# adfriend45/HYBRID9

Hardware: AMD Instinct MI355X
Metric: grid-cell-steps/sec at 0.5° global (1/2/4/8 GPUs) + achieved HBM GB/s (higher is better)
Workload: dtype f32

## Files before the change

hybrid9_amd/csrc/h9g.hip:

```cpp
#include <hip/hip_runtime.h>

#include <math.h>
#include <stdio.h>
#include <stdlib.h>
#include <string.h>

#include <algorithm>
#include <atomic>
#include <mutex>
#include <string>
#include <thread>
#include <vector>

#include "h9g_ctx.h"
#include "h9g_io.h"

static_assert(H9G_ERR_NOSNAP_K == H9G_ERR_NOSNAP, "kernel and ABI error codes");
static_assert(H9G_NDAILY == DAILY_ROWS, "the daily line of the ABI and of h9g_rows.h");

#define H9G_PF_ROWS 32
__global__ void __launch_bounds__(256) h9g_perm_forcing_kernel(int c0, int cend, int cpb, int nt, int n, size_t fvar,
                                                               size_t ds, size_t dvar, const int *__restrict__ perm,
                                                               const float *__restrict__ src, float *__restrict__ dst) {
  const unsigned nb = (unsigned)((cend - c0 + cpb - 1) / cpb), x = blockIdx.x % H9G_NXCD, j = blockIdx.x / H9G_NXCD;
// ... 1009 lines not shown
  for (int k = K_PAIR; k <= K_PROBE; k++)
    for (int j = 0; j < 3 && m < n; j++) out[m++] = ctx->kstat[k][j];
  if (reset)
    for (auto &row : ctx->kstat) row[0] = row[1] = row[2] = 0.0;
  return m;
}

#if defined(H9G_STAMPS)
static int stamps_report(h9g_ctx *ctx) {
  if (ctx->d_stamps && (ctx->kind == K_PAIR || ctx->kind == K_PAIR11 || ctx->kind == K_PAIR1)) {
    const size_t cw = (size_t)shape_info(kind_info(ctx->kind).shape).wave_cols, nw = (ctx->n + cw - 1) / cw;
    std::vector<unsigned> st(8 * nw);
    HIPCHK(hipMemcpy(st.data(), ctx->d_stamps, sizeof(unsigned) * 8 * nw, hipMemcpyDeviceToHost));
    double sum[8] = {0}, tot = 0;
    for (size_t w = 0; w < nw; w++)
      for (int k = 0; k < 8; k++) sum[k] += st[8 * w + k];
    const double steps = (double)nw * days_in_year(ctx->last_year) * ctx->cfg.nisurf;
    fprintf(stderr, "h9g stamps (cycles/wave/substep):");
    for (int k = 0; k < 8; k++) { fprintf(stderr, " p%d=%.0f", k, sum[k] / steps); tot += sum[k]; }
    fprintf(stderr, " total=%.0f\n", tot / steps);
    if (shape_info(ctx->stamp_shape).front()) {
      std::vector<unsigned> fs(8 * nw);
      HIPCHK(hipMemcpy(fs.data(), ctx->d_stamps + 8 * ctx->stamp_blocks, sizeof(unsigned) * 8 * nw, hipMemcpyDeviceToHost));
      double w = 0, f = 0;
      for (size_t k = 0; k < nw; k++) { w += fs[8 * k]; f += fs[8 * k + 1]; }
      fprintf(stderr, "h9g stamps, front waves (cycles/wave/substep): wait at barrier 1=%.0f front=%.0f\n", w / steps,
              f / steps);
    }
    std::vector<double> wt(nw, 0.0);
    for (size_t w = 0; w < nw; w++)
      for (int k = 0; k < 8; k++) wt[w] += st[8 * w + k];
    std::vector<double> ws(wt);
    std::sort(ws.begin(), ws.end());
    const double mean = tot / nw;
    fprintf(stderr, "h9g wave totals / mean: min %.3f p50 %.3f p90 %.3f p99 %.3f max %.3f\n", ws[0] / mean,
            ws[nw / 2] / mean, ws[nw * 9 / 10] / mean, ws[nw * 99 / 100] / mean, ws[nw - 1] / mean);
    double bx[8] = {0}, nx[8] = {0}, bs[4] = {0}, ns[4] = {0};
    for (size_t w = 0; w < nw; w++) {
      const size_t b = w / 4;
      bx[b % 8] += wt[w];
      nx[b % 8] += 1;
      bs[w % 4] += wt[w];
      ns[w % 4] += 1;
    }
    {
      const double cut90 = ws[nw * 9 / 10], cut50 = ws[nw / 2];
      double hi[8] = {0}, lo[8] = {0}, nh = 0, nl = 0;
      for (size_t w = 0; w < nw; w++) {
        if (wt[w] >= cut90) { nh++; for (int k = 0; k < 8; k++) hi[k] += st[8 * w + k]; }
        if (wt[w] <= cut50) { nl++; for (int k = 0; k < 8; k++) lo[k] += st[8 * w + k]; }
// ... 216 lines not shown
```

hybrid9_amd/csrc/h9g_pair.h:

```cpp
#pragma once
#include <type_traits>

#include "h9g_step.h"
#include "h9g_expr.h"
#if !defined(__HIPCC__) && !defined(__HIP__)
#define __device__
#define __forceinline__ inline
#endif

#ifndef H9G_EXACT_HOOK
#define H9G_EXACT_HOOK(k0, ns)
#endif
#if defined(H9G_COUNT_EXACT)
__device__ unsigned long long h9g_exact_count;
__device__ unsigned h9g_exact_wave[1 << 16];
#endif
namespace h9k {

enum : int {
  PF_TS = 0, PF_HKS, PF_BSW, PF_PSI,
  PF_NINVB,
  PF_ITS,
  PF_PTE,
  PF_C3,
// ... 8 lines not shown
  PS_LAI = PS_DAY + D_N,
  PS_LAIL, PS_PM, PS_PFM, PS_PLEN, PS_RDEPTH,
  PS_DR0,
  PS_DRS = PS_DR0 + 4 * DRP_N,
  PS_SVZWT = PS_DR0 + 2 * DR_N,
  PS_SVWA, PS_SVRNF, PS_SVERR, PS_SVNS,
  PS_SVEVAP,
  PS_N
};
enum : int { SV_ZWT = 0, SV_WA, SV_RNF, SV_ERR, SV_NS, SV_EVAP };
static_assert((PS_DAY + D_NUMC) % 2 == 0 && (PS_DAY + D_RAARAC) % 2 == 0 && (PS_DAY + D_DGRAC) % 2 == 0 &&
                  (PS_DAY + D_DRR) % 2 == 0 && (PS_DAY + D_RAC) % 2 == 0 && PS_DR0 % 2 == 0,
              "pair fields must start a row");

#ifndef H9G_EB_FAST
#define H9G_EB_FAST 1
#endif
#ifndef H9G_P1_TASKS
#define H9G_P1_TASKS 7
#endif
#ifndef H9G_P1_FRONT
#define H9G_P1_FRONT 1
#endif
enum : int { ROLE_ALL = 0, ROLE_FRONT = 1, ROLE_MAIN = 2 };
struct FrontRes {
  float qflx_surf, tran, evg, qflx_infl;
};

template <int K>
struct FV {
  float v[K];
};

H9K_HD float sel(int h, float a, float b) { return h ? b : a; }
H9K_HD double seld(int h, double a, double b) { return h ? b : a; }

H9K_HD float pair_swap(float v) {
#if defined(__HIP_DEVICE_COMPILE__)
  const int x = __builtin_bit_cast(int, v);
  return __builtin_bit_cast(float, __builtin_amdgcn_update_dpp(x, x, 0xB1, 0xF, 0xF, false));
#else
  return v;
#endif
}

template <int E>
H9K_HD float pair_bcast(float v) {
// ... 126 lines not shown
#endif
  }
};
#define H9G_PACE_ROWS 16384
__device__ __forceinline__ void pace_key(int &row, int &slot) {
#if defined(__HIP_DEVICE_COMPILE__)
  const unsigned hw = __builtin_amdgcn_s_getreg((31 << 11) | 4);
  const unsigned xcc = __builtin_amdgcn_s_getreg((3 << 11) | 20) & 15u;
  slot = (int)(hw & 15u);
  row = (int)(((((xcc * 8u + ((hw >> 13) & 7u)) * 2u + ((hw >> 12) & 1u)) * 16u + ((hw >> 8) & 15u)) * 4u) +
              ((hw >> 4) & 3u));
#else
  row = slot = 0;
#endif
}

template <int L>
constexpr int pair_resident() { return 3; }

template <int L, int S, int R = pair_resident<L>(), int F = 0>
struct PairStore {
  static constexpr int NT = L / 2;
  static constexpr bool kFront = F != 0;
  static_assert(!kFront || S == 2, "the front wave serves a one-column wave");
  static constexpr bool kRecip = true, kRts = L <= 8 || R <= 2 || S <= 22, kDayRecip = L <= 8 || R <= 2 || S <= 22;
  static constexpr bool kRtsHK = kRts;
  static constexpr int NPF = kRecip ? (kRts ? PF_SVH2O : PF_RTS0) : PF_RPSI0;
  static constexpr int NPS = kDayRecip ? PS_SVZWT : PS_DR0;
  static constexpr int TH0 = (NPF * NT + (NPS + 1) / 2) * S;
  enum : int {
    HO_SMP = TH0 + L, HO_H2O1 = HO_SMP + L, HO_ZWT, HO_GO, HO_PAD,
    HO_SURF, HO_TRAN, HO_EVG, HO_INFL, HO_END
  };
  static_assert((HO_END - TH0 - L) % 2 == 0, "whole rows");
  static constexpr int ROWS = NPF * NT + (NPS + 1) / 2 + (S == 2 ? NT : 0) + (kFront ? (HO_END - HO_SMP) / 2 : 0);
  static constexpr int GBLOCK = 65536;
  lds_float *self, *even;
  const lds_float *zt;
  float *svw;
  static constexpr int RESIDENT = R;
  Pacer pace;
  lds_float *wb;
  static constexpr int LANES = S;
  static constexpr bool kSpare = !(L >= 10 && R >= 3 && S >= 44);
  __device__ __forceinline__ void day_start(int day) const { pace.day_start(day, RESIDENT); }
  __device__ __forceinline__ float zi(int i) const { return zt[i]; }
  __device__ __forceinline__ float zim(int i) const { return zt[L + 2 + i]; }
  __device__ __forceinline__ double rdz_t(int i) const {
    return join_d(zt[2 * (L + 2) + 2 * i], zt[2 * (L + 2) + 2 * i + 1]);
  }
  __device__ __forceinline__ float lay(int p, int i) const {
    return even[(p * NT + ((i - 1) >> 1)) * S + ((i - 1) & 1)];
  }
  __device__ __forceinline__ void set_lay(int p, int i, float v) const {
    even[(p * NT + ((i - 1) >> 1)) * S + ((i - 1) & 1)] = v;
  }
  __device__ __forceinline__ float sc(int k) const { return even[(NPF * NT + (k >> 1)) * S + (k & 1)]; }
  __device__ __forceinline__ void set_sc(int k, float v) const {
// ... 328 lines not shown
    cs.set_lay(PF_NINVB, i, -one / bsw);
    cs.set_lay(PF_ITS, i, one / (ts + tsp));
    const float pte = psi * ts / e;
    cs.set_lay(PF_PTE, i, pte);
    cs.set_lay(PF_C3, i, pte / (g.zi(i) - g.zi(i - 1)));
    if constexpr (CS::kRecip) set_lay_d(cs, PF_RPSI0, i, recip64(-psi));
    if constexpr (CS::kRts) set_lay_d(cs, PF_RTS0, i, recip64(ts));
  }
  float mh = cs.lay(PF_HKS, 1);
  if (cs.lay(PF_HKS, 2) < mh) mh = cs.lay(PF_HKS, 2);
  if (cs.lay(PF_HKS, 3) < mh) mh = cs.lay(PF_HKS, 3);
  cs.set_sc(PS_MH3, mh);
  cs.set_sc(PS_TSDZ1, MAXF(zero, (cs.lay(PF_TS, 1) * g.dz(1))));
}

template <class M, class SP, class CS>
constexpr bool pair1_tasks() {
  if constexpr (H9G_P1_TASKS && SP::kSpare && CS::kSpare && !M::kExact)
    return CS::LANES == 2;
  else
    return false;
}

template <int L, class G, class M, class SP, class CS, class PR = NoProf, int ROLE = ROLE_ALL>
H9K_HD int hydrology_pair(const G &g, CS cs, const SP &sp0, St<L> &s, float &rnf_sum, float &errval,
                          M &m, PR &pr, FrontRes *fr = nullptr) {
  constexpr int NT = L / 2;
  const SP sp = L >= 10 ? sp0.fresh() : sp0;
  const float dt = g.dt();
  constexpr double r1000 = 1.0 / 1000.0;
  float zim[L + 1];
#pragma unroll
  for (int i = 1; i <= L; i++) zim[i] = g.zim(i);
  float *h2o = s.h2o, *smp = s.smp;
  float theta[L + 1];
  cs.launder();
#define TS(i) cs.lay(PF_TS, i)
#define HKS(i) cs.lay(PF_HKS, i)
#define BSW(i) cs.lay(PF_BSW, i)
#define PSI(i) cs.lay(PF_PSI, i)
#define LAYF(F, i) cs.lay(F, i)
#define ROOT(i) cs.lay(PF_ROOTR, i)
#define DC(F) cs.sc(PS_DAY + F)
#define OWN(p) sp.own(cs, p, t, h)

  float w0 = zero;
  if constexpr (ROLE == ROLE_FRONT) {
    theta[1] = m.div_d(h2o[1], g.thk(1), g.rthk(1));
    m.div_fix(theta[1], h2o[1], g.thk(1));
  } else {
  w0 = DC(D_FORC) * dt + s.wa;
  bool bad = false;
#pragma unroll
  for (int i = 1; i <= L; i++) {
    w0 = w0 + h2o[i];
    theta[i] = m.div_d(h2o[i], g.thk(i), g.rthk(i));
    bad |= m.div_bad(theta[i]);
  }
  if (__builtin_expect(bad, 0)) {
    H9G_BR(BR_THETA);
#pragma unroll
    for (int i = 1; i <= L; i++) m.div_fix(theta[i], h2o[i], g.thk(i));
  }
  }
  const float hkdepth = one / 2.5f;
  const float fff = 1.0f / hkdepth;
  const float frac_h2osfc = zero;
  float qflx_surf = zero, tran = zero, evg = zero, qflx_infl = zero;
  if constexpr (ROLE != ROLE_MAIN) {
  const float qflx_top_soil = DC(D_FORC);
  const float fsat = cs.sc(PS_FMAX) * m.expf(-0.5f * fff * s.zwt);
  qflx_surf = fsat * qflx_top_soil;
  float beta = zero;
  {
    float rb[L + 1];
    float *const out[1] = {rb};
    auto qb_x = [&](int t, int h) __attribute__((always_inline)) {
      return sel(h, smp[2 * t + 1] - g.zc(2 * t + 1), smp[2 * t + 2] - g.zc(2 * t + 2));
    };
    auto term = [&](int t, int h, float q) __attribute__((always_inline)) {
      float b = one - q;
      b = MINC(one, b);
      b = MAXF(zero, b);
      return FV<1>{{sp.own(cs, PF_ROOTR, t, h) * b}};
    };
    sp.template par_d<NT, 1, NT>(
        [&](int t, int h, bool &bad) __attribute__((always_inline)) -> FV<1> {
          const float q = m.div_d(qb_x(t, h), -150000.0f, 1.0 / -150000.0);
          bad |= m.div_bad(q);
          return term(t, h, q);
        },
        [&](int t, int h) __attribute__((always_inline)) -> FV<1> {
// ... 111 lines not shown
  tran = ftr.v[0];
  evg = fev.v[0];
  }
  float em1 = m.div(g.dz(1) * (theta[1] - watmin), dt, g.rdt()) - tran * ROOT(1);
  em1 = MAXF(zero, em1);
  evg = MINF(em1, evg);
  pr.flux(evg, tran);
  const float qflx_evap = evg;
  float qflx_in_soil = (one - frac_h2osfc) * (qflx_top_soil - qflx_surf);
  qflx_in_soil = qflx_in_soil - (one - frac_h2osfc) * qflx_evap;
  const float qinmax = (one - fsat) * cs.sc(PS_MH3);
  const float qflx_infl_excess = MAXF(zero, qflx_in_soil - (one - frac_h2osfc) * qinmax);
  qflx_infl = qflx_in_soil - qflx_infl_excess;
  qflx_surf = qflx_surf + qflx_infl_excess;
  }
  if constexpr (ROLE == ROLE_FRONT) {
    *fr = FrontRes{qflx_surf, tran, evg, qflx_infl};
    return 0;
  }
  float zwtmm = 1000.0f * s.zwt;
  const int jwt = jwt_of<L>(s.zwt, zim);
  const bool aq = (jwt == L);
  cs.launder();
  if constexpr (ROLE != ROLE_MAIN) pr.mark(1);

  float zq[L + 2];
  float hk[L + 1], dhkdw[L + 1], dsmpdw[L + 1];
  constexpr bool kTask = pair1_tasks<M, SP, CS>();
  FV<1> p0{{zero}}, p1{{zero}};
  FV<2> eA{{zero, zero}}, eS{{zero, zero}};
  bool picks = true, aq_task = false;
  float c_q[L + 1], c_1[L + 1], c_2[L + 1];
  bool flux_done = false;
  float rc_smp = zero, rc_zq = zero;
  {
    float *const outq[1] = {zq};
    float *const outk[4] = {hk, dhkdw, smp, dsmpdw};
    auto eq_exact = [&](int t, int h) __attribute__((always_inline)) -> FV<1> {
          H9G_BR(BR_EQX);
          const int i0 = 2 * t + 1;
          const int il = i0 + h;
          const float zlo = cs.zi(il - 1), zhi = cs.zi(il);
          const float ts = OWN(PF_TS), psi = OWN(PF_PSI);
          float vol_eq;
          if (zwtmm <= zlo) {
            vol_eq = ts;
          } else {
            const float expo = one + OWN(PF_NINVB);
            auto rp = [&]() __attribute__((always_inline)) {
              return join_d(OWN(PF_RPSI0), OWN(PF_RPSI1));
            };
            const bool inl = (zwtmm < zhi) && (zwtmm > zlo);
            const float n0 = ((-psi) + zwtmm - zlo), ni = (-psi + zwtmm - zhi);
            bool bq = false;
            float b0 = divr_d<CS::kRecip>(m, n0, -psi, rp, bq);
            float bi = divr_d<CS::kRecip>(m, ni, -psi, rp, bq);
            if (__builtin_expect(bq, 0)) {
              divr_fix<CS::kRecip>(m, b0, n0, -psi);
// ... 479 lines not shown
          };
          bool sq = false, sw = false;
          float q2 = divr_d<CS::kRts>(m, xn, TS(L), [&]() { return lay_d(cs, PF_RTS0, L); }, sq);
          float x = xof(q2);
          float pw = m.powf_d(x, -BSW(L), sw);
          if (__builtin_expect(sq | sw, 0)) {
            H9G_BR(BR_AQS);
            divr_fix<CS::kRts>(m, q2, xn, TS(L));
            x = xof(q2);
            pw = m.powf(x, -BSW(L));
          }
          const float z = smp_of(PSI(L), pw);
          return FV<2>{{z, dsmpdw_div(BSW(L), z, x, TS(L))}};
        },
        eA, eS);
  }
  }
  }
  const FV<1> pY = p1;
  zq[L + 1] = aq ? eA.v[0] : zero;
  const float smp1 = eS.v[0], dsmpdw1 = eS.v[1];
  cs.launder();
  pr.mark(3);
  if constexpr (ROLE == ROLE_MAIN) {
    cs.wg_sync();
    qflx_surf = cs.ho(CS::HO_SURF);
    tran = cs.ho(CS::HO_TRAN);
    evg = cs.ho(CS::HO_EVG);
    qflx_infl = cs.ho(CS::HO_INFL);
    pr.flux(evg, tran);
    pr.mark(1);
  }
  const float zcA = 0.5f * (zwtmm + g.zc(L));
  const float dzA = (jwt < L) ? g.dz(L) : zwtmm - g.zc(L);
  cs.launder();
  float dwat2[L + 2], GAM[L + 2];
  float BET = zero;
  double rbet = 0.0;
  int zero_pivot = 0;
  auto row = [&](int i, float am, float bm, float cm, float rm) __attribute__((always_inline)) {
    float x;
    if (i == 1) {
      BET = bm;
      x = rm;
    } else {
      BET = row_bet(am, bm, GAM[i]);
      if (BET == 0.0f && !zero_pivot) zero_pivot = i;
      x = row_x(am, rm, dwat2[i - 1]);
    }
    rbet = recip64(BET);
    dwat2[i] = m.div_d(x, BET, rbet);
    bool bad = m.div_bad(dwat2[i]);
    if (i <= L) {
      GAM[i + 1] = m.div_d(cm, BET, rbet);
      bad |= m.div_bad(GAM[i + 1]);
    }
    if (__builtin_expect(bad, 0)) {
      m.div_fix(dwat2[i], x, BET);
      if (i <= L) m.div_fix(GAM[i + 1], cm, BET);
    }
  };
  bool tri_ok = false;
  if constexpr (!M::kExact) {
    bool bad = false, zp = false;
    float qo[L + 1], d1[L + 1], d2[L + 1];
    auto flux3_f = [&](float hki, float num, float dsi, float dsn, float dhk, float den, double rden, int k,
                       bool &b) __attribute__((always_inline)) {
      qo[k] = m.div_d(flux_q(hki, num), den, rden);
      d1[k] = m.div_d(flux_d1(hki, num, dsi, dhk), den, rden);
      d2[k] = m.div_d(flux_d2(hki, num, dsn, dhk), den, rden);
      b |= m.div_bad(qo[k]) | m.div_bad(d1[k]) | m.div_bad(d2[k]);
    };
    if constexpr (kTask && (H9G_P1_TASKS & 2)) {
#pragma unroll
      for (int i = 1; i <= L; i++) {
        qo[i] = c_q[i];
        d1[i] = c_1[i];
        d2[i] = c_2[i];
      }
    }
    if (!kTask || __builtin_expect(!flux_done, 0)) {
#pragma unroll
    for (int i = 1; i <= L - 1; i++)
      flux3_f(hk[i], flux_num(smp[i + 1], smp[i], zq[i + 1], zq[i]), dsmpdw[i], dsmpdw[i + 1], dhkdw[i], g.den(i),
              g.rden(i), i, bad);
    qo[L] = d1[L] = d2[L] = zero;
// ... 42 lines not shown
      }
    };
    auto dzdt = [&](float dz) __attribute__((always_inline)) {
      const float q = m.div_d(dz, dt, g.rdt());
      bad |= m.div_bad(q);
      return q;
    };
    const float bm1 = dzdt(g.dz(1)) + d1[1];
    row_f(1, zero, bm1, d2[1], qflx_infl - qo[1] - tran * ROOT(1));
#pragma unroll
    for (int i = 2; i <= L - 1; i++)
      row_f(i, -d1[i - 1], dzdt(g.dz(i)) - d2[i - 1] + d1[i], d2[i], qo[i - 1] - qo[i] - tran * ROOT(i));
    row_f(L, -d1[L - 1], dzdt(g.dz(L)) - d2[L - 1] + (aq ? d1[L] : zero), aq ? d2[L] : zero,
          qo[L - 1] - (aq ? qo[L] : zero) - tran * ROOT(L));
    const float qA = dzdt(dzA);
    const float bmA = qA - d2[L] + zero;
    const float rmA = qo[L] - zero;
    row_f(L + 1, aq ? -d1[L] : zero, aq ? bmA : qA, zero, aq ? rmA : zero);
    if (__builtin_expect(bad | zp | (bm1 == 0.0f), 0)) {
      H9G_BR(BR_TRISWEEP);
      BET = zero;
      zero_pivot = 0;
      const float bm1x = m.div(g.dz(1), dt, g.rdt()) + d1[1];
      if (bm1x == 0.0f) { errval = bm1x; return 1; }
      row(1, zero, bm1x, d2[1], qflx_infl - qo[1] - tran * ROOT(1));
#pragma unroll
      for (int i = 2; i <= L - 1; i++)
        row(i, -d1[i - 1], m.div(g.dz(i), dt, g.rdt()) - d2[i - 1] + d1[i], d2[i], qo[i - 1] - qo[i] - tran * ROOT(i));
      if (!aq) {
        row(L, -d1[L - 1], m.div(g.dz(L), dt, g.rdt()) - d2[L - 1] + zero, zero, qo[L - 1] - zero - tran * ROOT(L));
        row(L + 1, zero, m.div(dzA, dt, g.rdt()), zero, zero);
      } else {
        row(L, -d1[L - 1], m.div(g.dz(L), dt, g.rdt()) - d2[L - 1] + d1[L], d2[L], qo[L - 1] - qo[L] - tran * ROOT(L));
        row(L + 1, -d1[L], m.div(dzA, dt, g.rdt()) - d2[L] + zero, zero, qo[L] - zero);
      }
      if (zero_pivot) { errval = (float)zero_pivot; return 2; }
    }
    tri_ok = true;
  }
  if (!tri_ok) {
  auto flux3 = [&](float hki, float num, float dsi, float dsn, float dhk, float den, double rden, float &qo,
                   float &d1, float &d2) __attribute__((always_inline)) {
    const float x0 = flux_q(hki, num), x1 = flux_d1(hki, num, dsi, dhk), x2 = flux_d2(hki, num, dsn, dhk);
    qo = m.div_d(x0, den, rden);
    d1 = m.div_d(x1, den, rden);
    d2 = m.div_d(x2, den, rden);
    if (__builtin_expect(m.div_bad(qo) | m.div_bad(d1) | m.div_bad(d2), 0)) {
      m.div_fix(qo, x0, den);
      m.div_fix(d1, x1, den);
      m.div_fix(d2, x2, den);
    }
  };
  float q_prev, dq0_prev, dq1_prev;
  {
    const float den = g.den(1);
    const double rden = g.rden(1);
    const float dzq = (zq[2] - zq[1]);
    const float num = (smp[2] - smp[1]) - dzq;
    float qout, dqodw1, dqodw2;
    flux3(hk[1], num, dsmpdw[1], dsmpdw[2], dhkdw[1], den, rden, qout, dqodw1, dqodw2);
    const float bm1 = m.div(g.dz(1), dt, g.rdt()) + dqodw1;
    if (bm1 == 0.0f) { errval = bm1; return 1; }
    row(1, zero, bm1, dqodw2, qflx_infl - qout - tran * ROOT(1));
    q_prev = qout; dq0_prev = dqodw1; dq1_prev = dqodw2;
  }
#pragma unroll
  for (int i = 2; i <= L - 1; i++) {
    const float den = g.den(i);
    const double rden = g.rden(i);
    const float dzq = zq[i + 1] - zq[i];
    const float num = (smp[i + 1] - smp[i]) - dzq;
    float qout, dqodw1, dqodw2;
    flux3(hk[i], num, dsmpdw[i], dsmpdw[i + 1], dhkdw[i], den, rden, qout, dqodw1, dqodw2);
    row(i, -dq0_prev, m.div(g.dz(i), dt, g.rdt()) - dq1_prev + dqodw1, dqodw2,
        q_prev - qout - tran * ROOT(i));
    q_prev = qout; dq0_prev = dqodw1; dq1_prev = dqodw2;
  }
  {
    constexpr int i = L;
    if (i > jwt) {
      const float qout = zero, dqodw1 = zero;
      row(i, -dq0_prev, m.div(g.dz(i), dt, g.rdt()) - dq1_prev + dqodw1, zero,
          q_prev - qout - tran * ROOT(i));
      row(i + 1, zero, m.div(dzA, dt, g.rdt()), zero, zero);
    } else {
      const float den = zcA - g.zc(i);
      const double rden = recip64(den);
      const float dzq = zq[i + 1] - zq[i];
      const float num = smp1 - smp[i] - dzq;
      float qout, dqodw1, dqodw2;
      flux3(hk[i], num, dsmpdw[i], dsmpdw1, dhkdw[i], den, rden, qout, dqodw1, dqodw2);
      row(i, -dq0_prev, m.div(g.dz(i), dt, g.rdt()) - dq1_prev + dqodw1, dqodw2,
          q_prev - qout - tran * ROOT(i));
      const float qout1 = zero, dqodw1b = zero;
      row(i + 1, -dqodw1, m.div(dzA, dt, g.rdt()) - dqodw2 + dqodw1b, zero, qout - qout1);
    }
  }
  if (zero_pivot) { errval = (float)zero_pivot; return 2; }
  }
#pragma unroll
  for (int i = L; i >= 1; i--) dwat2[i] = dwat2[i] - GAM[i + 1] * dwat2[i + 1];
#pragma unroll
  for (int i = 1; i <= L; i++) h2o[i] = h2o[i] + dwat2[i] * g.dz(i);
  cs.launder();
  pr.mark(4);
  auto s_y_base = [&](int i, float zmm) __attribute__((always_inline)) -> float {
    return one + divr<CS::kRecip>(m, zmm, -cs.lay(PF_PSI, i), [&]() { return lay_d(cs, PF_RPSI0, i); });
  };
  auto s_y_of = [&](int i, float pw) __attribute__((always_inline)) -> float {
    return MAXX(cs.lay(PF_TS, i) * (one - pw), 0.02f);
  };
  auto s_y_at = [&](int i, float zmm) __attribute__((always_inline)) -> float {
    return s_y_of(i, m.powf(s_y_base(i, zmm), cs.lay(PF_NINVB, i)));
  };
  float qcharge, sy_first = zero;
  if (jwt < L) {
    H9G_BR(BR_JWTCOL);
    const int j1 = jwt + 1;
    const float hks_j = cs.lay(PF_HKS, j1);
    float smp_m = zero, zq_m = zero, zc_j = zero;
    if constexpr (kTask && (H9G_P1_TASKS & 2)) {
      smp_m = rc_smp;
      zq_m = rc_zq;
#pragma unroll
      for (int i = 1; i <= L; i++)
        if (i == jwt) zc_j = g.zc(i);
    } else {
#pragma unroll
    for (int i = 1; i <= L; i++) {
      if (i == (jwt > 1 ? jwt : 1)) { smp_m = smp[i]; zq_m = zq[i]; }
      if (i == jwt) zc_j = g.zc(i);
    }
    }
    const float wh_zwt = zero;
    sy_first = s_y_of(jwt + 1, p1.v[0]);
    const float ka = hks_j * p0.v[0];
    const float smp1m = MAXC(smpmin, smp_m);
    const float wh = smp1m - zq_m;
    if (jwt == 0)
      qcharge = -ka * (wh_zwt - wh) / (zwtmm + one);
    else
      qcharge = -ka * (wh_zwt - wh) / ((zwtmm - zc_j) * 2.0f);
    qcharge = MAXC(-10.0f / dt, qcharge);
    qcharge = MINC(10.0f / dt, qcharge);
  } else {
    qcharge = m.div(dwat2[L + 1] * dzA, dt, g.rdt());
  }
  float rous = MAXX(TS(L) * (one - pY.v[0]), 0.02f);
  auto wdiv = [&](float x) __attribute__((always_inline)) {
    if constexpr (!M::kExact) {
      const float q = m.div_d(x, 1000.0f, r1000);
      m.special |= m.div_bad(q);
      return q;
    } else {
      return m.div(x, 1000.0f, r1000);
    }
  };
  int jwt2 = jwt;
  if (jwt == L) {
    s.wa = s.wa + qcharge * dt;
    s.zwt = s.zwt - m.div(qcharge * dt, 1000.0f, r1000) / rous;
  } else {
    float qcharge_tot = qcharge * dt;
    if (qcharge_tot > zero) {
      visit_layers(m, [&](int k) __attribute__((always_inline)) -> bool {
        const int i = jwt + 1 - k;
        const float s_y = k == 0 ? sy_first : s_y_at(i, zwtmm);
        float qcl = MINF(qcharge_tot, s_y * (zwtmm - cs.zi(i - 1)));
        qcl = MAXF(qcl, zero);
        if (s_y > zero) s.zwt = s.zwt - wdiv(qcl / s_y);
        qcharge_tot = qcharge_tot - qcl;
        return !(qcharge_tot <= zero || i == 1);
      });
    } else {
      visit_layers(m, [&](int k) __attribute__((always_inline)) -> bool {
        const int i = jwt + 1 + k;
        const float s_y = k == 0 ? sy_first : s_y_at(i, zwtmm);
        float qcl = MAXF(qcharge_tot, -s_y * (cs.zi(i) - zwtmm));
        qcl = MINF(qcl, zero);
        qcharge_tot = qcharge_tot - qcl;
        if (qcharge_tot >= zero) {
          s.zwt = s.zwt - wdiv(qcl / s_y);
          return false;
        }
        s.zwt = cs.zim(i);
        return i != L;
      });
      if (qcharge_tot > zero) {
        if (!aq) rous = s_y_at(L, zwtmm);
        s.zwt = s.zwt - wdiv(qcharge_tot) / rous;
      }
    }
    jwt2 = jwt_of<L>(s.zwt, zim);
  }
  cs.launder();
  pr.mark(5);
  zwtmm = 1000.0f * s.zwt;
  float rsub_top;
  const int jd = jwt2 < L ? jwt2 + 1 : L;
  FV<1> pR, pD;
  sp.template pick<1>(
      [&](int h) __attribute__((always_inline)) -> FV<1> {
        const int i = h ? jd : L;
        bool se = false, sq = false, sw = false;
        float ex = expf_fast(m, -fff * s.zwt, se);
        const float nb = -cs.lay(PF_PSI, i);
        float q = divr_d<CS::kRecip>(m, zwtmm, nb, [&]() { return lay_d(cs, PF_RPSI0, i); }, sq);
        float w = m.powf_d(one + q, cs.lay(PF_NINVB, i), sw);
        if (__builtin_expect(se | sq | sw, 0)) {
          H9G_BR(BR_BASE);
          if (se) ex = m.expf(-fff * s.zwt);
          divr_fix<CS::kRecip>(m, q, zwtmm, nb);
          w = m.powf(one + q, cs.lay(PF_NINVB, i));
        }
        rsub_top = 5.5E-3f * ex;
        return FV<1>{{w}};
      },
      pR, pD);
  rous = s_y_of(L, pR.v[0]);
  const float sy_drain = s_y_of(jd, pD.v[0]);
  int jwt3 = jwt2;
  if (jwt2 == L) {
    s.wa = s.wa - rsub_top * dt;
    s.zwt = s.zwt + m.div(rsub_top * dt, 1000.0f, r1000) / rous;
    h2o[L] = h2o[L] + MAXF(0.0f, (s.wa - 5000.0f));
    s.wa = MINF(s.wa, 5000.0f);
  } else {
    float rsub_top_tot = -rsub_top * dt;
    if (rsub_top_tot > zero) { errval = rsub_top_tot; return 3; }
    visit_layers(m, [&](int k) __attribute__((always_inline)) -> bool {
      const int i = jwt2 + 1 + k;
      const float s_y = k == 0 ? sy_drain : s_y_at(i, zwtmm);
      float rstl = MAXF(rsub_top_tot, -(s_y * (cs.zi(i) - zwtmm)));
      rstl = MINF(rstl, zero);
#pragma unroll
      for (int j = 1; j <= L; j++) {
        int hit = (j == i);
        opaque(hit);
        h2o[j] = hit ? h2o[j] + rstl : h2o[j];
      }
      rsub_top_tot = rsub_top_tot - rstl;
      if (rsub_top_tot >= zero) {
        s.zwt = s.zwt - wdiv(rstl / s_y);
        return false;
      }
      s.zwt = cs.zim(i);
      return i != L;
    });
    s.zwt = s.zwt - wdiv(rsub_top_tot) / rous;
    s.wa = s.wa + rsub_top_tot;
    jwt3 = jwt_of<L>(s.zwt, zim);
  }
  s.zwt = MAXF(0.0f, s.zwt);
  s.zwt = MINC(80.0f, s.zwt);
  cs.launder();
  pr.mark(6);
#pragma unroll
  for (int i = L; i >= 2; i--) {
    const float cap = MAXF(0.01f, TS(i)) * g.dz(i);
    const float xsi = MAXF(h2o[i] - cap, zero);
    h2o[i] = MINF(cap, h2o[i]);
    h2o[i - 1] = h2o[i - 1] + xsi;
  }
  const float xs1 = MAXF(MAXF(h2o[1], zero) - cs.sc(PS_TSDZ1), zero);
  h2o[1] = MINF(cs.sc(PS_TSDZ1), h2o[1]);
  float qflx_rsub_sat = m.div_d(xs1, dt, g.rdt());
  bool low = false;
#pragma unroll
  for (int i = 1; i <= L; i++) low |= h2o[i] < watmin;
  if (__builtin_expect(low | m.div_bad(qflx_rsub_sat), 0)) {
  H9G_BR(BR_WATMIN);
  m.div_fix(qflx_rsub_sat, xs1, dt);
#pragma unroll
  for (int i = 1; i <= L - 1; i++) {
    float xs = zero;
    if (h2o[i] < watmin) {
      xs = watmin - h2o[i];
// ... 22 lines not shown
        }
      }
    }
  }
  h2o[L] = h2o[L] + xs;
  rsub_top = rsub_top - m.div(xs, dt, g.rdt());
  }
  float w1 = ((1.0f - frac_h2osfc) * (qflx_surf + evg + tran) + rsub_top + qflx_rsub_sat) * dt + s.wa;
#pragma unroll
  for (int i = 1; i <= L; i++) w1 = w1 + h2o[i];
  pr.mark(7);
  if (absf(w1 - w0) > 0.1f) { errval = w1 - w0; return 4; }
  rnf_sum = rnf_sum + qflx_surf * dt;
  rnf_sum = rnf_sum + rsub_top * dt;
  return 0;
#undef TS
#undef HKS
#undef BSW
#undef PSI
#undef LAYF
#undef ROOT
#undef DC
#undef OWN
}

template <int L, class SP, class CS>
H9K_HD void save_day(const SP &sp, const CS &cs, const St<L> &s, float rnf_sum, int ns) {
  save_layers<L>(sp, cs, 0, s.h2o);
  save_layers<L>(sp, cs, 1, s.smp);
  cs.sv_set_sc(SV_ZWT, s.zwt);
  cs.sv_set_sc(SV_WA, s.wa);
  cs.sv_set_sc(SV_RNF, rnf_sum);
  cs.sv_set_sc(SV_NS, (float)ns);
}

template <int L, class G, class CS, bool EV = false>
H9K_RARE int substep_exact_pair(const G *g, CS cs, const uint64_t *e2, const double *l2, int ns) {
  cs.sv_sync();
  St<L> s;
#pragma unroll
  for (int i = 1; i <= L; i++) {
    s.h2o[i] = cs.sv_lay(0, i);
    s.smp[i] = cs.sv_lay(1, i);
  }
  s.zwt = cs.sv_sc(SV_ZWT);
  s.wa = cs.sv_sc(SV_WA);
// ... 16 lines not shown
  cs.sv_set_sc(SV_WA, s.wa);
  cs.sv_set_sc(SV_RNF, rnf);
  cs.sv_set_sc(SV_ERR, errval);
  cs.sv_set_sc(SV_NS, (float)(ns + 1));
  if constexpr (EV) cs.sv_set_sc(SV_EVAP, np.sum);
  cs.sv_sync();
  return code;
}

template <int L, class G, class SP, class CS, class PR>
H9K_HD int substep_pair(const G &g, CS cs, const SP &sp, St<L> &s, float &rnf_sum, float &errval,
                        const h9m::Tabs &T, PR &pr, int ns, bool snapped) {
  pr.mark(0);
  H9G_BR(BR_SUBSTEP);
#if defined(H9G_ISA_MARK) && defined(__HIP_DEVICE_COMPILE__)
  asm volatile("; h9g-substep");
#endif
  MathFast mf{T, false};
#if defined(H9G_FORCE_RERUN)
  const bool in_column = s.zwt <= g.zim(L);
#elif defined(H9G_FORCE_RERUN_ANY)
  const bool in_column = true;
#endif
  int code = hydrology_pair<L, G, MathFast, SP, CS, PR, CS::kFront ? ROLE_MAIN : ROLE_ALL>(g, cs, sp, s, rnf_sum,
                                                                                            errval, mf, pr);
#if defined(H9G_FORCE_RERUN)
  if (sp.act() && in_column && ns % H9G_FORCE_RERUN == H9G_FORCE_RERUN - 1) mf.special = true;
#elif defined(H9G_FORCE_RERUN_ANY)
  if (sp.act() && in_column && ns % H9G_FORCE_RERUN_ANY == H9G_FORCE_RERUN_ANY - 1) mf.special = true;
#endif
  if (__builtin_expect(sp.pair_any(mf.special), 0)) {
    H9G_BR(BR_RERUN);
    if (!snapped) {
      errval = (float)ns;
      return H9G_ERR_NOSNAP_K;
    }
#if defined(H9G_COUNT_EXACT) && defined(__HIP_DEVICE_COMPILE__)
    atomicAdd(&h9g_exact_count, 1ull);
    atomicAdd(&h9g_exact_wave[(blockIdx.x * 4 + (threadIdx.x >> 6)) & 0xffff], 1u);
#endif
    cs.launder();
    code = substep_exact_pair<L, G, CS, kEvap<PR>>(&g, cs, T.exp2, T.log2, ns);
    cs.launder();
#pragma unroll
    for (int i = 1; i <= L; i++) {
      s.h2o[i] = cs.sv_lay(0, i);
      s.smp[i] = cs.sv_lay(1, i);
    }
// ... 81 lines not shown
      o[4 * stride] = s.zwt;
      o[5 * stride] = s.wa;
      o[6 * stride] = s.LAI;
    }
    MonthsEt{M0 ? M0 + (A - A0) : nullptr, stride}.template day_end<L>(day, nt, A, as, rnf_sum, evap_sum);
  }
  H9K_HD void stop(int day, int nt, const gbl_float *A) const {
    if (!D0) return;
    gbl_float *o = D0 + (A - A0);
    const float nan = __builtin_nanf("");
    for (size_t k = (size_t)day * NREC; k < (size_t)nt * NREC; k++) o[k * stride] = nan;
  }
};
template <class MO>
constexpr bool kDays = std::is_same<MO, DaysEt>::value;

template <int L, class SP, class CS>
H9K_HD void front_post(const SP &sp, const CS &cs, const St<L> &s) {
#pragma unroll
  for (int t = 0; t < L / 2; t++) cs.set_ho(CS::HO_SMP + 2 * t + sp.h, sel(sp.h, s.smp[2 * t + 1], s.smp[2 * t + 2]));
  cs.set_ho(CS::HO_H2O1, s.h2o[1]);
  cs.set_ho(CS::HO_ZWT, s.zwt);
  cs.set_ho(CS::HO_GO, zero);
}
template <class CS>
H9K_HD void front_done(const CS &cs) {
  cs.set_ho(CS::HO_GO, one);
  cs.wg_sync();
}
template <int L, class G, class SP, class CS, class PR = NoProf>
H9K_HD void front_year_pair(const G &g, CS cs, const SP &sp, const h9m::Tabs &T, PR &&pr = PR()) {
  if (sp.spare) return;
  St<L> s{};
  float rnf_sum = zero, errval = zero;
  for (;;) {
    cs.wg_sync();
    cs.launder();
    if (lane0_get(cs.ho(CS::HO_GO)) != zero) break;
    pr.mark(0);
#pragma unroll
    for (int i = 1; i <= L; i++) s.smp[i] = cs.ho(CS::HO_SMP + i - 1);
    s.h2o[1] = cs.ho(CS::HO_H2O1);
    s.zwt = cs.ho(CS::HO_ZWT);
    MathFast mf{T, false};
    FrontRes fr;
    hydrology_pair<L, G, MathFast, SP, CS, PR, ROLE_FRONT>(g, cs, sp, s, rnf_sum, errval, mf, pr, &fr);
    pr.mark(1);
    cs.set_ho(CS::HO_SURF, fr.qflx_surf);
    cs.set_ho(CS::HO_TRAN, fr.tran);
    cs.set_ho(CS::HO_EVG, fr.evg);
    cs.set_ho(CS::HO_INFL, fr.qflx_infl);
    cs.wg_sync();
  }
}

template <int L, class G, class SP, class CS, bool Park = true, class PR = NoProf, class MO = NoMonths>
H9K_HD int cell_year_pair(const G &g, CS cs, const SP &sp, St<L> &s, const gbl_float *forc, size_t fday,
                          size_t fvar, int nt, int nisurf, int grow_on, gbl_float *acc, size_t astride,
                          int &eday, int &estep, float &errval, const h9m::Tabs &T, int raw = 0,
                          PR &&pr = PR(), MO mo = MO()) {
  enum { A_NPP = 0, A_PM, A_RNF, A_EVAP, A_TAS, A_RLDS, A_RSDS, A_HUSS, A_PS, A_PR, A_RHS,
         A_THETA, A_H2O = 11 + L };
  gbl_float *A = acc;
  const size_t as = astride;
  float rnf_sum = zero;
  const bool act = sp.act();
  if (act) {
#pragma unroll
    for (int k = 0; k < 12 + L; k++) A[k * as] = zero;
  }
  auto park = [&]() __attribute__((always_inline)) {
    if constexpr (Park) {
      if (!act) return;
      cs.set_sc(PS_LAI, s.LAI);
      cs.set_sc(PS_LAIL, s.LAI_litter);
// ... 232 lines not shown
```

hybrid9_amd/csrc/h9g_year.h:

```cpp
#pragma once
#include <hip/hip_runtime.h>

#include <stdint.h>
#include <stdio.h>

#include <type_traits>

#include "../../include/h9g.h"
#include "h9_math.h"
#include "h9g_geo.h"
#include "h9g_step.h"
#include "h9g_pair.h"
#include "h9g_rows.h"

using namespace h9k;

#define H9G_YBLOCK 64
#define H9G_PCPW 22
#define H9G_PLANES (2 * H9G_PCPW)
#define H9G_PWAVES 4
#define H9G_PCPW11 11

struct KArgs {
  int ncell;
// ... 115 lines not shown
    case K_SOLO: return {"solo", S_SOLO};
    case K_MIXED: return {"mixed", S_PAIR};
    case K_PAIR2: return {"pair2", S_PAIR2};
    case K_PAIR11: return {"pair11", S_PAIR11};
    case K_PAIR1: return {"pair1", S_PAIR1};
    default: return {"pair", S_PAIR};
  }
}

#define H9G_PAIR1_FRONT_MAX 512
inline Shape year_shape(int kind, size_t cells) {
  const Shape s = kind_info(kind).shape;
#if H9G_P1_FRONT
  if (s == S_PAIR1 && cells <= H9G_PAIR1_FRONT_MAX) return S_PAIR1F;
#endif
  return s;
}

template <int L, class G, int R, int C = H9G_PCPW, bool MON = false, bool FRONT = false, bool ET = false,
          bool DAY = false>
__device__ __forceinline__ void pair_body(const KArgs &a, const G &g, float *mon = nullptr, float *dayr = nullptr) {
  static_assert(!(MON && ET), "the ET kernels record months themselves");
  static_assert(!DAY || ET, "the day kernels are ET kernels");
  typedef PairStore<L, 2 * C, R, FRONT ? 1 : 0> PS;
  static_assert(!FRONT || C == 1, "the front wave serves a one-column wave");
  constexpr int NW = FRONT ? 1 : H9G_PWAVES;
  __shared__ uint64_t s_e2[32];
  __shared__ double s_l2[32];
  __shared__ float s_cell[NW][PS::ROWS * 2 * C];
  __shared__ float s_zt[zt_size<L>()];
  static_assert(sizeof(s_e2) + sizeof(s_l2) + sizeof(s_cell) + sizeof(s_zt) <= (size_t)PS::GBLOCK,
                "pair kernel LDS footprint exceeds the day-snapshot block");
  if (threadIdx.x == 0) fill_zt<L>(g, s_zt);
  load_tabs(s_e2, s_l2);
  const h9m::Tabs T = {s_e2, s_l2};
  const int wave = FRONT ? 0 : threadIdx.x >> 6, lane = threadIdx.x & 63;
  const bool front_wave = FRONT && __builtin_amdgcn_readfirstlane((int)(threadIdx.x >> 6)) != 0;
  const bool spare = lane >= 2 * C;
  if (spare && !PS::kSpare) return;
  const int h = lane & 1;
  const int slot0 = __builtin_amdgcn_readfirstlane(
      a.c0 + (int)(xcd_vwg(blockIdx.x, gridDim.x) * NW + wave) * C);
  const bool g2 = slot0 >= a.split;
  const int lim = g2 ? a.cend : a.bend;
  float *const st = g2 ? a.st2 : a.st;
  int *const err = g2 ? a.err2 : a.err;
  int *const hist = g2 ? nullptr : a.hist;
// ... 330 lines not shown
```

Baseline: 4.508 billion.

## Offload water-table recharge/drainage chain to the front wave in one-column pair kernel

Adds a ROLE_CHAIN side path in which the front wave, after its front work, runs the water-table recharge and subsurface-drainage chain. It reads the main wave's intermediate operands from LDS and writes back zwt, wa, drainage indices/amounts and error codes. The main wave (ROLE_MAINS) skips that chain, meets the front wave at an extra workgroup barrier, and applies the returned h2o adjustments when the column is not aquifer-bound. The aim is to take serial work off the main wave's critical path, at the cost of extra barriers, LDS rows and more code paths. Stamp reporting is also extended to show the new barrier and chain timings.

```diff
diff --git a/hybrid9_amd/csrc/h9g.hip b/hybrid9_amd/csrc/h9g.hip
--- a/hybrid9_amd/csrc/h9g.hip
+++ b/hybrid9_amd/csrc/h9g.hip
@@ -1055,10 +1055,19 @@
     if (shape_info(ctx->stamp_shape).front()) {
       std::vector<unsigned> fs(8 * nw);
       HIPCHK(hipMemcpy(fs.data(), ctx->d_stamps + 8 * ctx->stamp_blocks, sizeof(unsigned) * 8 * nw, hipMemcpyDeviceToHost));
-      double w = 0, f = 0;
-      for (size_t k = 0; k < nw; k++) { w += fs[8 * k]; f += fs[8 * k + 1]; }
-      fprintf(stderr, "h9g stamps, front waves (cycles/wave/substep): wait at barrier 1=%.0f front=%.0f\n", w / steps,
+      double w = 0, f = 0, w2 = 0, ch = 0, w3 = 0;
+      for (size_t k = 0; k < nw; k++) {
+        w += fs[8 * k];
+        f += fs[8 * k + 1];
+        w2 += fs[8 * k + 3] + fs[8 * k + 4];
+        ch += fs[8 * k + 5] + fs[8 * k + 6];
+        w3 += fs[8 * k + 7];
+      }
+      fprintf(stderr, "h9g stamps, front waves (cycles/wave/substep): wait at barrier 1=%.0f front=%.0f", w / steps,
               f / steps);
+      if (ch > 0)
+        fprintf(stderr, " wait at barrier 2=%.0f chain=%.0f wait at barrier 3=%.0f", w2 / steps, ch / steps, w3 / steps);
+      fprintf(stderr, "\n");
     }
     std::vector<double> wt(nw, 0.0);
     for (size_t w = 0; w < nw; w++)
diff --git a/hybrid9_amd/csrc/h9g_pair.h b/hybrid9_amd/csrc/h9g_pair.h
--- a/hybrid9_amd/csrc/h9g_pair.h
+++ b/hybrid9_amd/csrc/h9g_pair.h
@@ -54,7 +54,14 @@
 #ifndef H9G_P1_FRONT
 #define H9G_P1_FRONT 1
 #endif
-enum : int { ROLE_ALL = 0, ROLE_FRONT = 1, ROLE_MAIN = 2 };
+#ifndef H9G_P1_SIDE
+#define H9G_P1_SIDE 1
+#endif
+#if !H9G_P1_FRONT || (H9G_P1_TASKS & 3) != 3
+#undef H9G_P1_SIDE
+#define H9G_P1_SIDE 0
+#endif
+enum : int { ROLE_ALL = 0, ROLE_FRONT = 1, ROLE_MAIN = 2, ROLE_CHAIN = 3, ROLE_MAINS = 4 };
 struct FrontRes {
   float qflx_surf, tran, evg, qflx_infl;
 };
@@ -227,6 +234,7 @@
 struct PairStore {
   static constexpr int NT = L / 2;
   static constexpr bool kFront = F != 0;
+  static constexpr bool kSide = F == 2;
   static_assert(!kFront || S == 2, "the front wave serves a one-column wave");
   static constexpr bool kRecip = true, kRts = L <= 8 || R <= 2 || S <= 22, kDayRecip = L <= 8 || R <= 2 || S <= 22;
   static constexpr bool kRtsHK = kRts;
@@ -238,7 +246,13 @@
     HO_SURF, HO_TRAN, HO_EVG, HO_INFL, HO_END
   };
   static_assert((HO_END - TH0 - L) % 2 == 0, "whole rows");
-  static constexpr int ROWS = NPF * NT + (NPS + 1) / 2 + (S == 2 ? NT : 0) + (kFront ? (HO_END - HO_SMP) / 2 : 0);
+  enum : int {
+    HS_WA = HO_END, HS_P0, HS_PY, HS_RSMP, HS_RZQ, HS_PAD0,
+    HS_ZWT, HS_WAO, HS_RSUB, HS_JWT, HS_FLAG, HS_CODE, HS_ERRV, HS_I0, HS_R0, HS_I1, HS_R1, HS_PAD1, HS_END
+  };
+  static_assert((HS_END - HO_END) % 2 == 0, "whole rows");
+  static constexpr int ROWS =
+      NPF * NT + (NPS + 1) / 2 + (S == 2 ? NT : 0) + (kFront ? ((kSide ? HS_END : HO_END) - HO_SMP) / 2 : 0);
   static constexpr int GBLOCK = 65536;
   lds_float *self, *even;
   const lds_float *zt;
@@ -613,10 +627,24 @@
     return false;
 }
 
+template <class CS>
+constexpr int main_role() {
+  if constexpr (CS::kFront)
+    return CS::kSide ? ROLE_MAINS : ROLE_MAIN;
+  else
+    return ROLE_ALL;
+}
 template <int L, class G, class M, class SP, class CS, class PR = NoProf, int ROLE = ROLE_ALL>
 H9K_HD int hydrology_pair(const G &g, CS cs, const SP &sp0, St<L> &s, float &rnf_sum, float &errval,
                           M &m, PR &pr, FrontRes *fr = nullptr) {
   constexpr int NT = L / 2;
+  constexpr bool kMain = ROLE == ROLE_MAIN || ROLE == ROLE_MAINS;
+  constexpr bool kChain = ROLE == ROLE_CHAIN;
+#define STOP_RET(c)                                  \
+  {                                                  \
+    if constexpr (ROLE == ROLE_MAINS) cs.wg_sync();  \
+    return c;                                        \
+  }
   const SP sp = L >= 10 ? sp0.fresh() : sp0;
   const float dt = g.dt();
   constexpr double r1000 = 1.0 / 1000.0;
@@ -639,7 +667,7 @@
   if constexpr (ROLE == ROLE_FRONT) {
     theta[1] = m.div_d(h2o[1], g.thk(1), g.rthk(1));
     m.div_fix(theta[1], h2o[1], g.thk(1));
-  } else {
+  } else if constexpr (!kChain) {
   w0 = DC(D_FORC) * dt + s.wa;
   bool bad = false;
 #pragma unroll
@@ -658,7 +686,7 @@
   const float fff = 1.0f / hkdepth;
   const float frac_h2osfc = zero;
   float qflx_surf = zero, tran = zero, evg = zero, qflx_infl = zero;
-  if constexpr (ROLE != ROLE_MAIN) {
+  if constexpr (!kMain && !kChain) {
   const float qflx_top_soil = DC(D_FORC);
   const float fsat = cs.sc(PS_FMAX) * m.expf(-0.5f * fff * s.zwt);
   qflx_surf = fsat * qflx_top_soil;
@@ -816,7 +844,10 @@
   const int jwt = jwt_of<L>(s.zwt, zim);
   const bool aq = (jwt == L);
   cs.launder();
-  if constexpr (ROLE != ROLE_MAIN) pr.mark(1);
+  if constexpr (!kMain && !kChain) pr.mark(1);
+  if constexpr (kChain) {
+    if (aq) return 0;
+  }
 
   float zq[L + 2];
   float hk[L + 1], dhkdw[L + 1], dsmpdw[L + 1];
@@ -827,7 +858,14 @@
   float c_q[L + 1], c_1[L + 1], c_2[L + 1];
   bool flux_done = false;
   float rc_smp = zero, rc_zq = zero;
-  {
+  if constexpr (kChain) {
+    p0.v[0] = cs.ho(CS::HS_P0);
+    p1.v[0] = cs.ho(CS::HS_PY);
+    rc_smp = cs.ho(CS::HS_RSMP);
+    rc_zq = cs.ho(CS::HS_RZQ);
+    picks = false;
+    static_assert(!kChain || (kTask && (H9G_P1_TASKS & 2)), "the chain's operands come from the task rounds");
+  } else {
     float *const outq[1] = {zq};
     float *const outk[4] = {hk, dhkdw, smp, dsmpdw};
     auto eq_exact = [&](int t, int h) __attribute__((always_inline)) -> FV<1> {
@@ -1353,7 +1391,13 @@
   const float smp1 = eS.v[0], dsmpdw1 = eS.v[1];
   cs.launder();
   pr.mark(3);
-  if constexpr (ROLE == ROLE_MAIN) {
+  if constexpr (kMain) {
+    if constexpr (ROLE == ROLE_MAINS) {
+      cs.set_ho(CS::HS_P0, p0.v[0]);
+      cs.set_ho(CS::HS_PY, p1.v[0]);
+      cs.set_ho(CS::HS_RSMP, rc_smp);
+      cs.set_ho(CS::HS_RZQ, rc_zq);
+    }
     cs.wg_sync();
     qflx_surf = cs.ho(CS::HO_SURF);
     tran = cs.ho(CS::HO_TRAN);
@@ -1391,8 +1435,9 @@
       if (i <= L) m.div_fix(GAM[i + 1], cm, BET);
     }
   };
-  bool tri_ok = false;
-  if constexpr (!M::kExact) {
+  bool tri_ok = kChain;
+  if constexpr (kChain) dwat2[L + 1] = zero;
+  if constexpr (!M::kExact && !kChain) {
     bool bad = false, zp = false;
     float qo[L + 1], d1[L + 1], d2[L + 1];
     auto flux3_f = [&](float hki, float num, float dsi, float dsn, float dhk, float den, double rden, int k,
@@ -1481,7 +1526,7 @@
       BET = zero;
       zero_pivot = 0;
       const float bm1x = m.div(g.dz(1), dt, g.rdt()) + d1[1];
-      if (bm1x == 0.0f) { errval = bm1x; return 1; }
+      if (bm1x == 0.0f) { errval = bm1x; STOP_RET(1); }
       row(1, zero, bm1x, d2[1], qflx_infl - qo[1] - tran * ROOT(1));
 #pragma unroll
       for (int i = 2; i <= L - 1; i++)
@@ -1493,7 +1538,7 @@
         row(L, -d1[L - 1], m.div(g.dz(L), dt, g.rdt()) - d2[L - 1] + d1[L], d2[L], qo[L - 1] - qo[L] - tran * ROOT(L));
         row(L + 1, -d1[L], m.div(dzA, dt, g.rdt()) - d2[L] + zero, zero, qo[L] - zero);
       }
-      if (zero_pivot) { errval = (float)zero_pivot; return 2; }
+      if (zero_pivot) { errval = (float)zero_pivot; STOP_RET(2); }
     }
     tri_ok = true;
   }
@@ -1519,7 +1564,7 @@
     float qout, dqodw1, dqodw2;
     flux3(hk[1], num, dsmpdw[1], dsmpdw[2], dhkdw[1], den, rden, qout, dqodw1, dqodw2);
     const float bm1 = m.div(g.dz(1), dt, g.rdt()) + dqodw1;
-    if (bm1 == 0.0f) { errval = bm1; return 1; }
+    if (bm1 == 0.0f) { errval = bm1; STOP_RET(1); }
     row(1, zero, bm1, dqodw2, qflx_infl - qout - tran * ROOT(1));
     q_prev = qout; dq0_prev = dqodw1; dq1_prev = dqodw2;
   }
@@ -1555,14 +1600,27 @@
       row(i + 1, -dqodw1, m.div(dzA, dt, g.rdt()) - dqodw2 + dqodw1b, zero, qout - qout1);
     }
   }
-  if (zero_pivot) { errval = (float)zero_pivot; return 2; }
-  }
+  if (zero_pivot) { errval = (float)zero_pivot; STOP_RET(2); }
+  }
+  if constexpr (!kChain) {
 #pragma unroll
   for (int i = L; i >= 1; i--) dwat2[i] = dwat2[i] - GAM[i + 1] * dwat2[i + 1];
 #pragma unroll
   for (int i = 1; i <= L; i++) h2o[i] = h2o[i] + dwat2[i] * g.dz(i);
+  }
   cs.launder();
   pr.mark(4);
+  constexpr bool kOwn = ROLE != ROLE_MAINS;
+  float rsub_top;
+  int jwt3;
+  auto add_h2o = [&](int i, float v) __attribute__((always_inline)) {
+#pragma unroll
+    for (int j = 1; j <= L; j++) {
+      int hit = (j == i);
+      opaque(hit);
+      h2o[j] = hit ? h2o[j] + v : h2o[j];
+    }
+  };
   auto s_y_base = [&](int i, float zmm) __attribute__((always_inline)) -> float {
     return one + divr<CS::kRecip>(m, zmm, -cs.lay(PF_PSI, i), [&]() { return lay_d(cs, PF_RPSI0, i); });
   };
@@ -1573,7 +1631,7 @@
     return s_y_of(i, m.powf(s_y_base(i, zmm), cs.lay(PF_NINVB, i)));
   };
   float qcharge, sy_first = zero;
-  if (jwt < L) {
+  if (kOwn && jwt < L) {
     H9G_BR(BR_JWTCOL);
     const int j1 = jwt + 1;
     const float hks_j = cs.lay(PF_HKS, j1);
@@ -1619,7 +1677,7 @@
   if (jwt == L) {
     s.wa = s.wa + qcharge * dt;
     s.zwt = s.zwt - m.div(qcharge * dt, 1000.0f, r1000) / rous;
-  } else {
+  } else if (kOwn) {
     float qcharge_tot = qcharge * dt;
     if (qcharge_tot > zero) {
       visit_layers(m, [&](int k) __attribute__((always_inline)) -> bool {
@@ -1655,12 +1713,17 @@
   cs.launder();
   pr.mark(5);
   zwtmm = 1000.0f * s.zwt;
-  float rsub_top;
   const int jd = jwt2 < L ? jwt2 + 1 : L;
   FV<1> pR, pD;
   sp.template pick<1>(
       [&](int h) __attribute__((always_inline)) -> FV<1> {
         const int i = h ? jd : L;
+        if constexpr (!kOwn) {
+          if (!aq) {
+            rsub_top = zero;
+            return FV<1>{{zero}};
+          }
+        }
         bool se = false, sq = false, sw = false;
         float ex = expf_fast(m, -fff * s.zwt, se);
         const float nb = -cs.lay(PF_PSI, i);
@@ -1678,25 +1741,35 @@
       pR, pD);
   rous = s_y_of(L, pR.v[0]);
   const float sy_drain = s_y_of(jd, pD.v[0]);
-  int jwt3 = jwt2;
+  jwt3 = jwt2;
   if (jwt2 == L) {
     s.wa = s.wa - rsub_top * dt;
     s.zwt = s.zwt + m.div(rsub_top * dt, 1000.0f, r1000) / rous;
+    if constexpr (kChain) {
+      cs.set_ho(CS::HS_I0, (float)L);
+      cs.set_ho(CS::HS_R0, MAXF(0.0f, (s.wa - 5000.0f)));
+    } else {
     h2o[L] = h2o[L] + MAXF(0.0f, (s.wa - 5000.0f));
+    }
     s.wa = MINF(s.wa, 5000.0f);
-  } else {
+  } else if (kOwn) {
     float rsub_top_tot = -rsub_top * dt;
-    if (rsub_top_tot > zero) { errval = rsub_top_tot; return 3; }
+    if (rsub_top_tot > zero) { errval = rsub_top_tot; STOP_RET(3); }
     visit_layers(m, [&](int k) __attribute__((always_inline)) -> bool {
       const int i = jwt2 + 1 + k;
       const float s_y = k == 0 ? sy_drain : s_y_at(i, zwtmm);
       float rstl = MAXF(rsub_top_tot, -(s_y * (cs.zi(i) - zwtmm)));
       rstl = MINF(rstl, zero);
+      if constexpr (kChain) {
+        cs.set_ho(CS::HS_I0 + 2 * k, (float)i);
+        cs.set_ho(CS::HS_R0 + 2 * k, rstl);
+      } else {
 #pragma unroll
       for (int j = 1; j <= L; j++) {
         int hit = (j == i);
         opaque(hit);
         h2o[j] = hit ? h2o[j] + rstl : h2o[j];
+      }
       }
       rsub_top_tot = rsub_top_tot - rstl;
       if (rsub_top_tot >= zero) {
@@ -1712,6 +1785,31 @@
   }
   s.zwt = MAXF(0.0f, s.zwt);
   s.zwt = MINC(80.0f, s.zwt);
+  if constexpr (kChain) {
+    cs.set_ho(CS::HS_RSUB, rsub_top);
+    cs.set_ho(CS::HS_JWT, (float)jwt3);
+    pr.mark(6);
+    return 0;
+  }
+  if constexpr (ROLE == ROLE_MAINS) {
+    cs.wg_sync();
+    if (!aq) {
+      pr.mark(5);
+      s.zwt = cs.ho(CS::HS_ZWT);
+      s.wa = cs.ho(CS::HS_WAO);
+      rsub_top = cs.ho(CS::HS_RSUB);
+      jwt3 = (int)cs.ho(CS::HS_JWT);
+      const int scode = (int)cs.ho(CS::HS_CODE);
+      if (__builtin_expect(scode != 0, 0)) {
+        errval = cs.ho(CS::HS_ERRV);
+        return scode;
+      }
+      m.special |= cs.ho(CS::HS_FLAG) != zero;
+      const int i0 = (int)cs.ho(CS::HS_I0), i1 = (int)cs.ho(CS::HS_I1);
+      if (i0) add_h2o(i0, cs.ho(CS::HS_R0));
+      if (i1) add_h2o(i1, cs.ho(CS::HS_R1));
+    }
+  }
   cs.launder();
   pr.mark(6);
 #pragma unroll
@@ -1780,6 +1878,7 @@
 #undef ROOT
 #undef DC
 #undef OWN
+#undef STOP_RET
 }
 
 template <int L, class SP, class CS>
@@ -1842,8 +1941,7 @@
 #elif defined(H9G_FORCE_RERUN_ANY)
   const bool in_column = true;
 #endif
-  int code = hydrology_pair<L, G, MathFast, SP, CS, PR, CS::kFront ? ROLE_MAIN : ROLE_ALL>(g, cs, sp, s, rnf_sum,
-                                                                                            errval, mf, pr);
+  int code = hydrology_pair<L, G, MathFast, SP, CS, PR, main_role<CS>()>(g, cs, sp, s, rnf_sum, errval, mf, pr);
 #if defined(H9G_FORCE_RERUN)
   if (sp.act() && in_column && ns % H9G_FORCE_RERUN == H9G_FORCE_RERUN - 1) mf.special = true;
 #elif defined(H9G_FORCE_RERUN_ANY)
@@ -1971,6 +2069,7 @@
   cs.set_ho(CS::HO_H2O1, s.h2o[1]);
   cs.set_ho(CS::HO_ZWT, s.zwt);
   cs.set_ho(CS::HO_GO, zero);
+  if constexpr (CS::kSide) cs.set_ho(CS::HS_WA, s.wa);
 }
 template <class CS>
 H9K_HD void front_done(const CS &cs) {
@@ -2000,6 +2099,21 @@
     cs.set_ho(CS::HO_EVG, fr.evg);
     cs.set_ho(CS::HO_INFL, fr.qflx_infl);
     cs.wg_sync();
+    if constexpr (CS::kSide) {
+      cs.launder();
+      s.wa = cs.ho(CS::HS_WA);
+      cs.set_ho(CS::HS_I0, zero);
+      cs.set_ho(CS::HS_I1, zero);
+      MathFast mc{T, false};
+      const int code = hydrology_pair<L, G, MathFast, SP, CS, PR, ROLE_CHAIN>(g, cs, sp, s, rnf_sum, errval, mc, pr);
+      cs.set_ho(CS::HS_ZWT, s.zwt);
+      cs.set_ho(CS::HS_WAO, s.wa);
+      cs.set_ho(CS::HS_FLAG, mc.special ? one : zero);
+      cs.set_ho(CS::HS_CODE, (float)code);
+      cs.set_ho(CS::HS_ERRV, errval);
+      cs.wg_sync();
+      pr.mark(7);
+    }
   }
 }
 
diff --git a/hybrid9_amd/csrc/h9g_year.h b/hybrid9_amd/csrc/h9g_year.h
--- a/hybrid9_amd/csrc/h9g_year.h
+++ b/hybrid9_amd/csrc/h9g_year.h
@@ -161,7 +161,7 @@
 __device__ __forceinline__ void pair_body(const KArgs &a, const G &g, float *mon = nullptr, float *dayr = nullptr) {
   static_assert(!(MON && ET), "the ET kernels record months themselves");
   static_assert(!DAY || ET, "the day kernels are ET kernels");
-  typedef PairStore<L, 2 * C, R, FRONT ? 1 : 0> PS;
+  typedef PairStore<L, 2 * C, R, FRONT ? (H9G_P1_SIDE ? 2 : 1) : 0> PS;
   static_assert(!FRONT || C == 1, "the front wave serves a one-column wave");
   constexpr int NW = FRONT ? 1 : H9G_PWAVES;
   __shared__ uint64_t s_e2[32];
```

Measured after the change: 4.625 billion (median of 6 runs). 1.03x the previous value.
